# ablab/stringdecomposer

Hardware: AMD Instinct MI355X
Metric: decomposed read-bp/sec (whole node) at 12 monomers x 50kb reads (higher is better)
Workload: dtype u16

## Files before the change

stringdecomposer_amd/csrc/sd_fast_fill.hpp:

```cpp
#pragma once

#include <hip/hip_runtime.h>

#include <algorithm>
#include <climits>
#include <cstdlib>
#include <type_traits>

#include "sd_fast.hpp"
#include "sd_fast_dev.hpp"

namespace sd {

#define SD_FILL_NW_MAX 16
template <int P, bool RANKED, int CF, int FL = P, bool ONE = false, int FLS = 0>
__global__ __launch_bounds__(SD_FILL_NW_MAX * 64, 4) void sd_fast_fill(
    const ChunkDesc* __restrict__ chunks, int n_chunks, const uint32_t* __restrict__ bases2,
    const uint32_t* __restrict__ nmask, const uint32_t* __restrict__ table,
    const uint32_t* __restrict__ lane_consts, ScoreArgs sc, uint32_t Hx, unsigned long long levels, int32_t* __restrict__ Bout,
    int32_t* __restrict__ argV, uint32_t* __restrict__ ckpt, int32_t* __restrict__ ckbase,
    int* __restrict__ queue, const int* __restrict__ order, const uint32_t* __restrict__ cendoff,
    const uint32_t* __restrict__ crank) {
    constexpr int P4 = (P + 3) & ~3;
    extern __shared__ __attribute__((aligned(16))) uint32_t lds[];
    constexpr int TBL = 5 * P4 * 64;
    constexpr bool F16 = CF == CF_F16, U16 = CF == CF_U16;
    using CO = CellOps<CF>;
    constexpr uint32_t NEGC = CO::NEG;
    for (int idx = threadIdx.x * 4; idx < TBL; idx += blockDim.x * 4) {
        uint4 q = *reinterpret_cast<const uint4*>(&table[idx]);
        if constexpr (F16) {
            q.x = CO::from_i16x2(q.x); q.y = CO::from_i16x2(q.y);
            q.z = CO::from_i16x2(q.z); q.w = CO::from_i16x2(q.w);
        }
        if constexpr (U16) {
            const uint32_t tm = lane_consts[((idx >> 2) & 63) * FAST_LANE_WORDS + FLC_TMPL];
            const int tpad = min(min(sc.match, sc.mismatch) - sc.del - sc.ins, 0);
            const int plo = (tm & 0xffffu) == 0xffffu ? 0 : tpad, phi = (tm >> 16) == 0xffffu ? 0 : tpad;
            auto cv = [&](uint32_t w) {
                const int lo = (int)(short)(w & 0xffffu), hi = (int)w >> 16;
                return spair(lo <= -30000 ? plo : lo, hi <= -30000 ? phi : hi);
            };
            q.x = cv(q.x); q.y = cv(q.y); q.z = cv(q.z); q.w = cv(q.w);
        }
        *reinterpret_cast<uint4*>(&lds[idx]) = q;
    }
    __syncthreads();

    const int wave = __builtin_amdgcn_readfirstlane((int)(threadIdx.x >> 6));
    const int nw = (int)(blockDim.x >> 6);
    const int lane = threadIdx.x & 63;
    (void)wave; (void)nw; (void)levels;
    const int H = Hx & 0xff;
    const bool bperm_ok = (Hx >> 8) & 1;
    FairShare fair;
    fair.init(reinterpret_cast<int*>(lds + TBL), wave, nw, lane, queue, n_chunks);
    ChunkSched sched;
    sched.init(queue, order, n_chunks);
    for (int c = sched.next(); c >= 0; c = sched.next()) {
    const ChunkDesc cd = chunks[c];
    const int n = cd.n;
    ReadStream rs;
    rs.init(bases2 + cd.woff, cd.noff >= 0 ? nmask + cd.noff : nullptr, n);
    bool bperm_scan = bperm_ok && (!fair.drained || ((Hx >> 9) & 1));

    const uint32_t* lc = lane_consts + lane * FAST_LANE_WORDS;
    const uint32_t startMask = lc[FLC_STARTMASK];
    const uint32_t contMask = lc[FLC_CONTMASK];
    const uint32_t cont2Mask = lc[FLC_CONT2];
    const uint32_t oneMask = ONE ? lc[FLC_ONE] : 0u;
    const uint32_t endOffPlan = lc[FLC_ENDOFF];
    constexpr bool HRED = F16 || U16;
    constexpr bool SLOT_RUNS = U16 && FLS > 0;
    const uint32_t endOffRaw = pk_adds(RANKED ? cendoff[(size_t)c * 64 + lane] : lc[FLC_ENDALL], pack2(sc.del));
    const uint32_t endOff = HRED ? CO::from_i16x2(endOffRaw)
                                 : CO::from_i16x2(RANKED ? cendoff[(size_t)c * 64 + lane] : endOffPlan);
    const uint32_t rank2 = RANKED ? crank[(size_t)c * 64 + lane] : 0u;
    const uint32_t row0adj = CO::from_i16x2(lc[FLC_ROW0]);
    const uint32_t ins2 = CO::splat(sc.ins);
    uint32_t planeMask = 0xffffffffu, endMask = 0xffffffffu, notStart = ~startMask;
    if constexpr (U16) {
        const uint32_t tm = lc[FLC_TMPL];
        planeMask = ((tm & 0xffffu) == 0xffffu ? 0u : 0xffffu) | ((tm >> 16) == 0xffffu ? 0u : 0xffff0000u);
        endMask = ((int)(short)(endOffRaw & 0xffffu) <= -30000 ? 0u : 0xffffu) | (((int)endOffRaw >> 16) <= -30000 ? 0u : 0xffff0000u);
        asm volatile("" : "+v"(planeMask), "+v"(endMask), "+v"(notStart));
    }

    int32_t* Bc = Bout + cd.row0 + (uint64_t)c;
    uint32_t* ck = ckpt + (uint64_t)cd.pad * (uint64_t)(P * 64) + lane;
    int32_t* ckb = ckbase + cd.pad;

    uint32_t L[P];
    uint32_t tb[P4];
    uint32_t K = NEGC;
    int base = 0, Brel = 0, tp = 0;
    uint32_t bdel16 = 0;
    int accBV = 0;
    int flush_at = min(n, 64);

    typedef uint32_t u32x4_t __attribute__((ext_vector_type(4)));
    using lds_u4 = __attribute__((address_space(3))) const u32x4_t;
    const uint32_t lds_lane = (uint32_t)(uintptr_t)(__attribute__((address_space(3))) const uint32_t*)lds + lane * 16;
    auto load_table = [&](int r, uint32_t& after) {
        uint32_t addr = lds_lane + (uint32_t)(r * (P4 * 256));
        asm volatile("" : "+v"(addr), "+v"(after));
        lds_u4* t = (lds_u4*)(uintptr_t)addr;
#pragma unroll
        for (int c4 = 0; c4 < P4 / 4; ++c4) {
            const u32x4_t q = t[c4 * 64];
            tb[4 * c4 + 0] = q.x; tb[4 * c4 + 1] = q.y; tb[4 * c4 + 2] = q.z; tb[4 * c4 + 3] = q.w;
        }
    };
    const int idle4 = (int)(((Hx >> 16) & 63u) << 2);
    int bp1 = (contMask & 0xffffu) ? (lane - 1) << 2 : idle4;
    int bp2 = (cont2Mask & 0xffffu) ? (lane - 2) << 2 : idle4;
    asm volatile("" : "+v"(bp1), "+v"(bp2));
    auto excl_scan = [&](uint32_t a) {
        uint32_t inc = a;
        if (bperm_scan) {
            inc = CO::mx(inc, (uint32_t)__builtin_amdgcn_ds_bpermute(bp1, (int)inc));
            inc = CO::mx(inc, (uint32_t)__builtin_amdgcn_ds_bpermute(bp2, (int)inc));
            return (uint32_t)__builtin_amdgcn_ds_bpermute(bp1, (int)inc);
        }
        if (H <= 4) {
            inc = CO::mx(inc, bfi(contMask, lane_up(inc, 1), NEGC));
            inc = CO::mx(inc, bfi(cont2Mask, lane_up(lane_up(inc, 1), 1), NEGC));
        } else {
            for (int h = 1; h < H; ++h) inc = CO::mx(a, bfi(contMask, lane_up(inc, 1), NEGC));
        }
        return bfi(contMask, lane_up(inc, 1), NEGC);
    };
    auto reduce_ends = [&](uint32_t Eend, int row) {
        if constexpr (HRED) {
            uint32_t val = CO::add(Eend, endOff);
            if constexpr (U16 && RANKED) val &= endMask;
            uint32_t m;
            asm("v_max_f16_sdwa %0, %1, %1 dst_sel:DWORD dst_unused:UNUSED_PAD src0_sel:WORD_0 src1_sel:WORD_1\n\t"
                "s_nop 1\n\t"
                "v_max_f16_dpp %0, %0, %0 row_shr:1 row_mask:0xf bank_mask:0xf\n\t"
                "s_nop 1\n\t"
                "v_max_f16_dpp %0, %0, %0 row_shr:2 row_mask:0xf bank_mask:0xf\n\t"
                "s_nop 1\n\t"
                "v_max_f16_dpp %0, %0, %0 row_shr:4 row_mask:0xf bank_mask:0xf\n\t"
                "s_nop 1\n\t"
                "v_max_f16_dpp %0, %0, %0 row_shr:8 row_mask:0xf bank_mask:0xf\n\t"
                "s_nop 1\n\t"
                "v_max_f16_dpp %0, %0, %0 row_bcast:15 row_mask:0xa bank_mask:0xf\n\t"
                "s_nop 1\n\t"
                "v_max_f16_dpp %0, %0, %0 row_bcast:31 row_mask:0xc bank_mask:0xf"
                : "=&v"(m) : "v"(val));
            const uint32_t b16 = (uint32_t)__builtin_amdgcn_readlane((int)m, 63) & 0xffffu;
            unsigned long long mlo, mhi;
            asm("v_cmp_eq_f16_e64 %0, %1, %2" : "=s"(mlo) : "v"(val), "s"(b16));
            asm("v_cmp_eq_f16_sdwa %0, %1, %2 src0_sel:WORD_1 src1_sel:WORD_0" : "=s"(mhi) : "v"(val), "s"(b16));
            if constexpr (RANKED) {
                if (__popcll(mlo) + __popcll(mhi) > 1) {
                    const int klo = ((mlo >> lane) & 1ull) ? (int)(rank2 & 0xffffu) : 0x7fff;
                    const int khi = ((mhi >> lane) & 1ull) ? (int)(rank2 >> 16) : 0x7fff;
                    const int kmin = -wave_max(-min(klo, khi));
                    mlo = __ballot(klo == kmin);
                    mhi = __ballot(khi == kmin);
                }
            }
            const int v = mlo ? __builtin_ctzll(mlo) : 64 + __builtin_ctzll(mhi);
            bdel16 = b16;
            const int slot = (row - 1) & 63;
            acc_put(accBV, (int)((b16 << 7) | (uint32_t)v), slot);
            if (row == flush_at) {
                flush_at = min(n, row + 64);
                asm volatile("");
                const uint32_t w = (uint32_t)accBV;
                const int bi = U16 ? (int)(w >> 7) - U16_BIAS : (int)(float)__builtin_bit_cast(_Float16, (unsigned short)(w >> 7));
                const int tpl = tp - (slot - lane);
                const int Bv = base + bi - sc.del + tpl * sc.ins;
                if (lane <= slot) Bc[row - slot + lane] = (int)(((uint32_t)Bv << 7) | (w & 127u));
            }
            return;
        }
        const uint32_t val = CO::add(Eend, endOff);
        int lo, hi;
        CO::to_int(val, lo, hi);
        const int b = wave_max(max(lo, hi));
        unsigned long long mlo, mhi;
        if (RANKED) {
            mlo = __ballot(lo == b);
            mhi = __ballot(hi == b);
            if (__popcll(mlo) + __popcll(mhi) > 1) {
                const int klo = lo == b ? (int)(rank2 & 0xffffu) : 0x7fff;
                const int khi = hi == b ? (int)(rank2 >> 16) : 0x7fff;
                const int kmin = -wave_max(-min(klo, khi));
                mlo = __ballot(klo == kmin);
                mhi = __ballot(khi == kmin);
            }
        } else {
            mlo = __ballot(lo == b);
            mhi = __ballot(hi == b);
        }
        const int v = mlo ? (__ffsll((long long)mlo) - 1) : (64 + __ffsll((long long)mhi) - 1);
        Brel = b + tp * sc.ins;
        const int slot = (row - 1) & 63;
        acc_put(accBV, (int)(((uint32_t)(base + Brel) << 7) | (uint32_t)v), slot);
        if (row == flush_at) {
            flush_at = min(n, row + 64);
            if (lane <= slot) Bc[row - slot + lane] = accBV;
        }
    };

    uint32_t pin = 0;
    load_table(rs.code(0), pin);
    rs.advance(0);
    if constexpr (U16) {
        L[0] = (tb[0] + row0adj + U16_BIAS2) & planeMask;
#pragma unroll
        for (int q = 1; q < P; ++q) L[q] = CO::mx(L[q - 1], (tb[q] + ins2 + U16_BIAS2) & planeMask);
    } else {
    L[0] = CO::add(tb[0], row0adj);
#pragma unroll
    for (int q = 1; q < P; ++q) L[q] = CO::mx(L[q - 1], CO::add(tb[q], ins2));
    }
    int rcur = rs.code(1);
    int rprev = 4;
    (void)rprev;
    load_table(rcur, L[P - 1]);
    rs.advance(1);
    std::conditional_t<U16, U16Guard<P>, F16Guard<P>> guard;
    if constexpr (F16) {
        guard.start(L[P - 1], sc.guard_lim);
        guard.check_low(L);
    }
    if constexpr (U16) {
        guard.start(sc.guard_lim);
        guard.check_low(L, planeMask);
    }
    const uint32_t a0 = ONE ? bfi(oneMask, L[0], L[P - 1]) : L[P - 1];
    if constexpr (HRED) reduce_ends(a0, 1);
    K = excl_scan(a0);
    uint32_t Eend = CO::mx(a0, K);
    if constexpr (!HRED) reduce_ends(Eend, 1);

    for (int i = 1; i < n;) {
        if ((i & (FAST_R - 1)) == 0) {
            fair.update(n - i);
            bperm_scan = bperm_ok && (!fair.drained || ((Hx >> 9) & 1));
            if ((i & (127 >> ((Hx >> 11) & 1))) == 0) {
                if constexpr (F16)
                    Brel = __builtin_amdgcn_readfirstlane((int)(float)__builtin_bit_cast(_Float16, (unsigned short)bdel16)) -
                           sc.del + tp * sc.ins;
                if constexpr (U16) Brel = (int)bdel16 - U16_BIAS - sc.del + tp * sc.ins;
                const uint32_t d2 = U16 ? pack2(-(Brel - tp * sc.ins)) : CO::splat(F16 ? -(Brel - tp * sc.ins) : Brel - tp * sc.ins);
                base += Brel;
                Brel = 0;
                tp = 0;
                if constexpr (F16) bdel16 = __builtin_amdgcn_readfirstlane((int)(CO::splat(sc.del) & 0xffffu));
                if constexpr (U16) bdel16 = (uint32_t)(U16_BIAS + sc.del);
                if constexpr (U16) {
                    typedef unsigned short u2_t __attribute__((ext_vector_type(2)));
                    auto shift = [](uint32_t x, uint32_t d) {
                        return __builtin_bit_cast(uint32_t, __builtin_bit_cast(u2_t, x) + __builtin_bit_cast(u2_t, d));
                    };
                    const uint32_t d2m = d2 & planeMask;
                    guard.check_high(L);
                    K = shift(K, d2m & notStart);
#pragma unroll
                    for (int s = 0; s < P; ++s) L[s] = shift(L[s], d2m);
                    guard.check_low(L, planeMask);
                } else if constexpr (F16) {
                    guard.check_high(L);
                    K = bfi(startMask, NEGC, CO::add(K, d2));
                    Eend = CO::add(Eend, d2);
#pragma unroll
                    for (int s = 0; s < P; ++s) L[s] = CO::add(L[s], d2);
                    guard.check_low(L);
                } else {
                K = bfi(startMask, NEG2, pk_subs(K, d2));
                Eend = pk_subs(Eend, d2);
#pragma unroll
                for (int s = 0; s < P; ++s) L[s] = pk_subs(L[s], d2);
                }
            }
            const int q = (i / FAST_R) - 1;
#pragma unroll
            for (int s = 0; s < P; ++s) ck[(uint64_t)q * (P * 64) + s * 64] = CO::mx(L[s], K);
            if (lane == 0) ckb[q] = base + tp * sc.ins;
        }
        const int iend = min(n, (i | (FAST_R - 1)) + 1);
        for (; i < iend; ++i) {
        uint32_t KB;
        if constexpr (HRED) {
            asm("v_pk_max_f16 %0, %1, %2 op_sel_hi:[1,0]" : "=v"(KB) : "v"(K), "s"(bdel16));
            if constexpr (U16) KB &= planeMask;
        } else {
            KB = CO::mx(K, CO::splat(Brel + sc.del - tp * sc.ins));
        }
        const uint32_t w0 = U16 ? (L[0] & notStart) : bfi(startMask, NEGC, L[0]);
        uint32_t u_[P], v_[P], c_[P];
        uint32_t run = 0;
        if constexpr (HRED) {
            if constexpr (FLS > 0) {
                constexpr int FL3 = FL - 3 * FLS > 1 ? FL - 3 * FLS : 1;
                constexpr int FL2 = FL - 2 * FLS > FL3 ? FL - 2 * FLS : FL3;
                constexpr int FL1 = FL - FLS > FL2 ? FL - FLS : FL2;
                const int lv = (int)(levels >> (2 * (5 * rprev + rcur))) & 3;
#pragma unroll
                for (int q = 1; q <= FL3 && q < P; ++q) L[q - 1] = CO::mx(L[q - 1], KB);
                if (lv <= 2) {
#pragma unroll
                    for (int q = FL3 + 1; q <= FL2 && q < P; ++q) L[q - 1] = CO::mx(L[q - 1], KB);
                }
                if (lv <= 1) {
#pragma unroll
                    for (int q = FL2 + 1; q <= FL1 && q < P; ++q) L[q - 1] = CO::mx(L[q - 1], KB);
                }
                if (lv == 0) {
#pragma unroll
                    for (int q = FL1 + 1; q <= FL && q < P; ++q) L[q - 1] = CO::mx(L[q - 1], KB);
                }
            }
            const uint32_t w0f = FLS > 0 ? (U16 ? (L[0] & notStart) : bfi(startMask, NEGC, L[0])) : w0;
            if constexpr (SLOT_RUNS) {
#pragma unroll
                for (int q = P - 1; q >= 1; --q) asm volatile("v_add_u32 %0, %0, %1" : "+v"(tb[q]) : "v"(L[q - 1]));
                asm volatile("v_add_u32 %0, %0, %1" : "+v"(tb[0]) : "v"(KB));
                asm volatile("v_pk_maximum3_f16 %0, %1, %2, %3" : "=v"(L[0]) : "v"(tb[0]), "v"(w0f), "v"(K));
#pragma unroll
                for (int q = 1; q < P; ++q)
                    asm volatile("v_pk_maximum3_f16 %0, %1, %2, %0" : "+v"(L[q]) : "v"(L[q - 1]), "v"(tb[q]));
            } else {
#pragma unroll
            for (int s = 0; s < P + 4; ++s) {
                if (s >= 4) {
                    const int q = s - 4;
                    L[q] = q == 0 ? CO::mx3(v_[0], w0f, K) : CO::mx3(L[q - 1], v_[q], L[q]);
                }
                if (s >= 2 && s - 2 < P) {
                    const int q = s - 2;
                    v_[q] = CO::add(u_[q], tb[q]);
                }
                if (s < P) {
                    const int q = s;
                    if (q == 0) u_[q] = KB;
                    else if (FLS == 0 && q <= FL) u_[q] = CO::mx(L[q - 1], KB);
                    else u_[q] = L[q - 1];
                }
                __builtin_amdgcn_sched_barrier(0);
            }
            }
            (void)c_; (void)run; (void)u_; (void)v_;
        } else {
#pragma unroll
        for (int s = 0; s < P + 3; ++s) {
            if (s >= 3) {
                const int q = s - 3;
                run = q == 0 ? c_[0] : pk_max(run, c_[q]);
                L[q] = run;
            }
            if (s >= 2 && s - 2 < P) {
                const int q = s - 2;
                c_[q] = pk_max(v_[q], q == 0 ? w0 : L[q]);
            }
            if (s >= 1 && s - 1 < P) {
                const int q = s - 1;
                v_[q] = pk_adds(u_[q], tb[q]);
            }
            if (s < P) {
                const int q = s;
                u_[q] = q == 0 ? KB : q <= FL ? pk_max(L[q - 1], KB) : L[q - 1];
            }
            __builtin_amdgcn_sched_barrier(0);
        }
        }
        rprev = rcur;
        rcur = rs.code(i + 1);
        load_table(rcur, L[P - 1]);
        rs.advance(i + 1);
        uint32_t a = HRED ? L[P - 1] : CO::mx(L[P - 1], K);
        if constexpr (ONE) a = bfi(oneMask, L[0], a);
        ++tp;
        if constexpr (HRED) {
            uint32_t t1 = 0;
            if (bperm_scan) t1 = (uint32_t)__builtin_amdgcn_ds_bpermute(bp1, (int)a);
            reduce_ends(a, i + 1);
            if (bperm_scan) {
                const uint32_t i1 = CO::mx(a, t1);
                const uint32_t i2 = CO::mx(i1, (uint32_t)__builtin_amdgcn_ds_bpermute(bp2, (int)i1));
                K = (uint32_t)__builtin_amdgcn_ds_bpermute(bp1, (int)i2);
            } else {
                K = excl_scan(a);
            }
        } else {
            K = excl_scan(a);
            Eend = CO::mx(a, K);
            reduce_ends(Eend, i + 1);
        }
        }
    }
    if constexpr (HRED) {
        guard.check_high(L);
        guard.finish(sc.guard_flag);
    }
    }
    fair.leave();
}


}
```

Before: 3.991 billion.

## Software-pipeline table load and end reduction, pre-add tail lanes early in fill loop

For the SLOT_RUNS path, the row-code advance and table offset are computed at the top of each iteration. The LDS table load for the next row is now interleaved between the split phases of the DPP end-of-row max reduction and the bpermute scan, so LDS latency overlaps with cross-lane work. The tail columns beyond FL get their table adds applied early in a pre_add step after the previous row, and the shift on renormalisation is extended to keep them consistent. This adds scheduling barriers and extra live registers, which could raise register pressure or cause subtle correctness risk.

```diff
diff --git a/stringdecomposer_amd/csrc/sd_fast_fill.hpp b/stringdecomposer_amd/csrc/sd_fast_fill.hpp
--- a/stringdecomposer_amd/csrc/sd_fast_fill.hpp
+++ b/stringdecomposer_amd/csrc/sd_fast_fill.hpp
@@ -101,8 +101,8 @@
     typedef uint32_t u32x4_t __attribute__((ext_vector_type(4)));
     using lds_u4 = __attribute__((address_space(3))) const u32x4_t;
     const uint32_t lds_lane = (uint32_t)(uintptr_t)(__attribute__((address_space(3))) const uint32_t*)lds + lane * 16;
-    auto load_table = [&](int r, uint32_t& after) {
-        uint32_t addr = lds_lane + (uint32_t)(r * (P4 * 256));
+    auto load_table_at = [&](uint32_t off, uint32_t& after) {
+        uint32_t addr = lds_lane + off;
         asm volatile("" : "+v"(addr), "+v"(after));
         lds_u4* t = (lds_u4*)(uintptr_t)addr;
 #pragma unroll
@@ -110,6 +110,12 @@
             const u32x4_t q = t[c4 * 64];
             tb[4 * c4 + 0] = q.x; tb[4 * c4 + 1] = q.y; tb[4 * c4 + 2] = q.z; tb[4 * c4 + 3] = q.w;
         }
+    };
+    auto load_table = [&](int r, uint32_t& after) { load_table_at((uint32_t)(r * (P4 * 256)), after); };
+    constexpr int PRE_FROM = SLOT_RUNS ? (FL < P - 1 ? FL : P - 1) + 1 : P;
+    auto pre_add = [&]() {
+#pragma unroll
+        for (int q = P - 1; q >= PRE_FROM; --q) asm volatile("v_add_u32 %0, %0, %1" : "+v"(tb[q]) : "v"(L[q - 1]));
     };
     const int idle4 = (int)(((Hx >> 16) & 63u) << 2);
     int bp1 = (contMask & 0xffffu) ? (lane - 1) << 2 : idle4;
@@ -130,13 +136,18 @@
         }
         return bfi(contMask, lane_up(inc, 1), NEGC);
     };
-    auto reduce_ends = [&](uint32_t Eend, int row) {
-        if constexpr (HRED) {
-            uint32_t val = CO::add(Eend, endOff);
-            if constexpr (U16 && RANKED) val &= endMask;
+    auto ends_val = [&](uint32_t Eend) {
+        uint32_t val = CO::add(Eend, endOff);
+        if constexpr (U16 && RANKED) val &= endMask;
+        return val;
+    };
+    auto ends_join = [&](uint32_t val) {
             uint32_t m;
-            asm("v_max_f16_sdwa %0, %1, %1 dst_sel:DWORD dst_unused:UNUSED_PAD src0_sel:WORD_0 src1_sel:WORD_1\n\t"
-                "s_nop 1\n\t"
+            asm("v_max_f16_sdwa %0, %1, %1 dst_sel:DWORD dst_unused:UNUSED_PAD src0_sel:WORD_0 src1_sel:WORD_1" : "=v"(m) : "v"(val));
+            return m;
+    };
+    auto ends_max = [&](uint32_t m) {
+            asm("s_nop 1\n\t"
                 "v_max_f16_dpp %0, %0, %0 row_shr:1 row_mask:0xf bank_mask:0xf\n\t"
                 "s_nop 1\n\t"
                 "v_max_f16_dpp %0, %0, %0 row_shr:2 row_mask:0xf bank_mask:0xf\n\t"
@@ -148,8 +159,10 @@
                 "v_max_f16_dpp %0, %0, %0 row_bcast:15 row_mask:0xa bank_mask:0xf\n\t"
                 "s_nop 1\n\t"
                 "v_max_f16_dpp %0, %0, %0 row_bcast:31 row_mask:0xc bank_mask:0xf"
-                : "=&v"(m) : "v"(val));
-            const uint32_t b16 = (uint32_t)__builtin_amdgcn_readlane((int)m, 63) & 0xffffu;
+                : "+v"(m));
+            return (uint32_t)__builtin_amdgcn_readlane((int)m, 63) & 0xffffu;
+    };
+    auto ends_put = [&](uint32_t val, uint32_t b16, int row) {
             unsigned long long mlo, mhi;
             asm("v_cmp_eq_f16_e64 %0, %1, %2" : "=s"(mlo) : "v"(val), "s"(b16));
             asm("v_cmp_eq_f16_sdwa %0, %1, %2 src0_sel:WORD_1 src1_sel:WORD_0" : "=s"(mhi) : "v"(val), "s"(b16));
@@ -175,6 +188,11 @@
                 const int Bv = base + bi - sc.del + tpl * sc.ins;
                 if (lane <= slot) Bc[row - slot + lane] = (int)(((uint32_t)Bv << 7) | (w & 127u));
             }
+    };
+    auto reduce_ends = [&](uint32_t Eend, int row) {
+        if constexpr (HRED) {
+            const uint32_t val = ends_val(Eend);
+            ends_put(val, ends_max(ends_join(val)), row);
             return;
         }
         const uint32_t val = CO::add(Eend, endOff);
@@ -237,6 +255,7 @@
     K = excl_scan(a0);
     uint32_t Eend = CO::mx(a0, K);
     if constexpr (!HRED) reduce_ends(Eend, 1);
+    pre_add();
 
     for (int i = 1; i < n;) {
         if ((i & (FAST_R - 1)) == 0) {
@@ -263,6 +282,8 @@
                     K = shift(K, d2m & notStart);
 #pragma unroll
                     for (int s = 0; s < P; ++s) L[s] = shift(L[s], d2m);
+#pragma unroll
+                    for (int q = PRE_FROM; q < P; ++q) tb[q] = shift(tb[q], d2m);
                     guard.check_low(L, planeMask);
                 } else if constexpr (F16) {
                     guard.check_high(L);
@@ -284,7 +305,25 @@
             if (lane == 0) ckb[q] = base + tp * sc.ins;
         }
         const int iend = min(n, (i | (FAST_R - 1)) + 1);
+        const int trips_word = bperm_scan;
+        auto trips_on = [&]() {
+            int t = trips_word;
+            asm volatile("" : "+s"(t));
+            return t != 0;
+        };
+        (void)trips_on;
         for (; i < iend; ++i) {
+        int lv = 0;
+        uint32_t toff = 0;
+        (void)lv; (void)toff;
+        if constexpr (FLS > 0) lv = (int)(levels >> (2 * (5 * rprev + rcur))) & 3;
+        if constexpr (SLOT_RUNS) {
+            rprev = rcur;
+            rcur = rs.code(i + 1);
+            rs.advance(i + 1);
+            toff = (uint32_t)(rcur * (P4 * 256));
+            asm volatile("" : "+s"(lv), "+s"(toff));
+        }
         uint32_t KB;
         if constexpr (HRED) {
             asm("v_pk_max_f16 %0, %1, %2 op_sel_hi:[1,0]" : "=v"(KB) : "v"(K), "s"(bdel16));
@@ -300,7 +339,6 @@
                 constexpr int FL3 = FL - 3 * FLS > 1 ? FL - 3 * FLS : 1;
                 constexpr int FL2 = FL - 2 * FLS > FL3 ? FL - 2 * FLS : FL3;
                 constexpr int FL1 = FL - FLS > FL2 ? FL - FLS : FL2;
-                const int lv = (int)(levels >> (2 * (5 * rprev + rcur))) & 3;
 #pragma unroll
                 for (int q = 1; q <= FL3 && q < P; ++q) L[q - 1] = CO::mx(L[q - 1], KB);
                 if (lv <= 2) {
@@ -319,7 +357,7 @@
             const uint32_t w0f = FLS > 0 ? (U16 ? (L[0] & notStart) : bfi(startMask, NEGC, L[0])) : w0;
             if constexpr (SLOT_RUNS) {
 #pragma unroll
-                for (int q = P - 1; q >= 1; --q) asm volatile("v_add_u32 %0, %0, %1" : "+v"(tb[q]) : "v"(L[q - 1]));
+                for (int q = PRE_FROM - 1; q >= 1; --q) asm volatile("v_add_u32 %0, %0, %1" : "+v"(tb[q]) : "v"(L[q - 1]));
                 asm volatile("v_add_u32 %0, %0, %1" : "+v"(tb[0]) : "v"(KB));
                 asm volatile("v_pk_maximum3_f16 %0, %1, %2, %3" : "=v"(L[0]) : "v"(tb[0]), "v"(w0f), "v"(K));
 #pragma unroll
@@ -368,6 +406,35 @@
             }
             __builtin_amdgcn_sched_barrier(0);
         }
+        }
+        if constexpr (SLOT_RUNS) {
+            uint32_t a = L[P - 1];
+            if constexpr (ONE) a = bfi(oneMask, L[0], a);
+            ++tp;
+            uint32_t t1, i1;
+            if (trips_on()) t1 = (uint32_t)__builtin_amdgcn_ds_bpermute(bp1, (int)a);
+            __builtin_amdgcn_sched_barrier(0);
+            const uint32_t val = ends_val(a);
+            uint32_t m = ends_join(val);
+            load_table_at(toff, m);
+            __builtin_amdgcn_sched_barrier(0);
+            uint32_t b16 = ends_max(m);
+            asm volatile("" : "+s"(b16));
+            asm volatile("" : : "v"(tb[P4 - 1]));
+            if (trips_on()) {
+                i1 = CO::mx(a, t1);
+                t1 = (uint32_t)__builtin_amdgcn_ds_bpermute(bp2, (int)i1);
+            }
+            __builtin_amdgcn_sched_barrier(0);
+            ends_put(val, b16, i + 1);
+            pre_add();
+            if (trips_on()) {
+                const uint32_t i2 = CO::mx(i1, t1);
+                K = (uint32_t)__builtin_amdgcn_ds_bpermute(bp1, (int)i2);
+            } else {
+                K = excl_scan(a);
+            }
+            continue;
         }
         rprev = rcur;
         rcur = rs.code(i + 1);
```

After: 4.033 billion, median of 6. 1.01x the previous value.
